# qirui-chen/RGA3-release

Measured on AMD Instinct MI355X. Metric: video-QA samples/sec (fwd+bwd) at 7B/16-frame — full RGA3 training step (Qwen2.5-VL-7B + SAM2-L + mask losses + AdamW), higher is better.
Workload: dtype bf16

## Files before the change

### rga3-release_amd/csrc/attn_args.h

```cpp
#pragma once
#include "common.h"

namespace rga3 {

struct AttnArgs {
    const unsigned short* q;
    const unsigned short* k;
    const unsigned short* v;
    unsigned short* o;
    float* lse;
    const int* cu_q;
    const int* cu_k;
    long q_st, q_sh, k_st, k_sh, v_st, v_sh, o_st, o_sh;
    int Hq, Hkv, D;
    long total_q;
    float scale_log2;
    int causal;
    float* split_o;
    float* split_lse;
    int nsplit;
    int bq_shift, bk_shift;
    const float* rope_cos;
    const float* rope_sin;
    const float* rope_kcos;
    const float* rope_ksin;
    int gx;
};

int launch_causal32(const AttnArgs& a, int nseg, int max_q, hipStream_t st);

}
```

### rga3-release_amd/csrc/attn_bwd.hip

```cpp
#include "common.h"

#include <mutex>
#include <set>

namespace rga3 {

struct AttnBwdArgs {
    const unsigned short *q, *k, *v, *o, *dout;
    unsigned short *dq, *dk, *dv;
    const float* lse;
    float* delta;
    const int *cu_q, *cu_k;
    long q_st, q_sh, k_st, k_sh, v_st, v_sh, o_st, o_sh, do_st, do_sh, dq_st, dq_sh, dk_st, dk_sh, dv_st, dv_sh;
    int Hq, Hkv, D;
    long total_q;
    float scale, scale_log2;
    int causal;
    float* dkv_ws;
    long total_k;
    int gx, gy;
};

constexpr int BT = 64;

template <int DP, int QT, int NWAVE, bool PAIR>
__global__ __launch_bounds__(64 * NWAVE) void attn_bwd_dq_kernel(AttnBwdArgs p) {
    constexpr int NT = 64 * NWAVE;
    constexpr int BLOCK_M = NWAVE * QT * 16;
    constexpr int CH = DP / 8;
    constexpr int STRIDE = DP * 2 + 32;
    constexpr int DS = DP / 32, DT = DP / 16;
    constexpr int LOADS = (BT * CH) / NT;
    static_assert((BT * CH) % NT == 0, "tile chunks must divide evenly over threads");

    extern __shared__ __attribute__((aligned(16))) char smem[];
    char* Ks = smem;
    char* Vs = smem + BT * STRIDE;

    const int tid = threadIdx.x, lane = tid & 63;
    const int wid = __builtin_amdgcn_readfirstlane(tid >> 6);
    const int g = lane >> 4, c = lane & 15;
    const Wg3 wg = xcd_decode3(p.gx, p.gy);
    const int seg = wg.z, hq = wg.y;
    const int hk = hq / (p.Hq / p.Hkv);
    const int qs = p.cu_q[seg], Lq = p.cu_q[seg + 1] - qs;
    const int ks = p.cu_k[seg], Lk = p.cu_k[seg + 1] - ks;
    const int shift = Lk - Lq;
    const int nqb = (Lq + BLOCK_M - 1) / BLOCK_M;
    int qb_first = wg.x, qb_second = -1;
    if constexpr (PAIR) {
        qb_first = nqb - 1 - wg.x;
        qb_second = wg.x;
        if (qb_second > qb_first) return;
        if (qb_second == qb_first) qb_second = -1;
    } else if (qb_first >= nqb) {
        return;
    }
    for (int pass = 0; pass < (PAIR ? 2 : 1); ++pass) {
    const int qbi = pass == 0 ? qb_first : qb_second;
    if (qbi < 0) break;
    if (pass == 1) __syncthreads();
    const int qb0 = qbi * BLOCK_M;
    const int qw0 = qb0 + wid * (QT * 16);

    bf16x8 qf[QT][DS], dof[QT][DS];
    float lse2[QT], dl[QT];
#pragma unroll
    for (int t = 0; t < QT; ++t) {
        const int qi = qw0 + t * 16 + c;
        const bool ok = qi < Lq;
#pragma unroll
        for (int ds = 0; ds < DS; ++ds) {
            const int d = ds * 32 + g * 8;
            u32x4 z = {0u, 0u, 0u, 0u}, y = {0u, 0u, 0u, 0u};
            if (ok && d < p.D) {
                z = *(const u32x4*)(p.q + (long)(qs + qi) * p.q_st + (long)hq * p.q_sh + d);
                y = *(const u32x4*)(p.dout + (long)(qs + qi) * p.do_st + (long)hq * p.do_sh + d);
            }
            qf[t][ds] = __builtin_bit_cast(bf16x8, z);
            dof[t][ds] = __builtin_bit_cast(bf16x8, y);
        }
        lse2[t] = ok ? p.lse[(long)hq * p.total_q + qs + qi] * 1.4426950408889634f : 0.f;
    }
#pragma unroll
    for (int t = 0; t < QT; ++t) {
        const int qi = qw0 + t * 16 + c;
        const bool ok = qi < Lq;
        float dp = 0.f;
#pragma unroll
        for (int ds = 0; ds < DS; ++ds) {
            const int d = ds * 32 + g * 8;
            if (ok && d < p.D) {
                const u32x4 ov = *(const u32x4*)(p.o + (long)(qs + qi) * p.o_st + (long)hq * p.o_sh + d);
                const u32x4 dv = __builtin_bit_cast(u32x4, dof[t][ds]);
#pragma unroll
                for (int i = 0; i < 4; ++i) {
                    dp += __uint_as_float(ov[i] << 16) * __uint_as_float(dv[i] << 16);
                    dp += __uint_as_float(ov[i] & 0xffff0000u) * __uint_as_float(dv[i] & 0xffff0000u);
                }
            }
        }
        dp += __shfl_xor(dp, 16, 64);
        dp += __shfl_xor(dp, 32, 64);
        dl[t] = ok ? dp : 0.f;
        if (ok && g == 0) p.delta[(long)hq * p.total_q + qs + qi] = dp;
    }

    f32x4 dqacc[QT][DT];
#pragma unroll
    for (int t = 0; t < QT; ++t)
#pragma unroll
        for (int d = 0; d < DT; ++d) dqacc[t][d] = f32x4{0.f, 0.f, 0.f, 0.f};

    int kv_end = Lk;
    if (p.causal) kv_end = min(Lk, qb0 + BLOCK_M + shift);
    if (kv_end < 0) kv_end = 0;
    const int ntiles = (kv_end + BT - 1) / BT;

    u32x4 kreg[LOADS], vreg[LOADS];
    auto load_tile = [&](int kt) {
#pragma unroll
        for (int i = 0; i < LOADS; ++i) {
            const int idx = tid + i * NT;
            const int r = idx / CH, ch = idx % CH;
            const int key = kt * BT + r;
            u32x4 zk = {0u, 0u, 0u, 0u}, zv = {0u, 0u, 0u, 0u};
            if (key < Lk && ch * 8 < p.D) {
                zk = *(const u32x4*)(p.k + (long)(ks + key) * p.k_st + (long)hk * p.k_sh + ch * 8);
                zv = *(const u32x4*)(p.v + (long)(ks + key) * p.v_st + (long)hk * p.v_sh + ch * 8);
            }
            kreg[i] = zk;
            vreg[i] = zv;
        }
    };
    auto store_tile = [&]() {
#pragma unroll
        for (int i = 0; i < LOADS; ++i) {
            const int idx = tid + i * NT;
            const int r = idx / CH, ch = idx % CH;
            *(u32x4*)(Ks + r * STRIDE + ch * 16) = kreg[i];
            *(u32x4*)(Vs + r * STRIDE + ch * 16) = vreg[i];
        }
    };

    if (ntiles > 0) load_tile(0);
    for (int kt = 0; kt < ntiles; ++kt) {
        __syncthreads();
        store_tile();
        __syncthreads();
        if (kt + 1 < ntiles) load_tile(kt + 1);
        const int k0 = kt * BT;
        const bool need_mask = (k0 + BT > Lk) || (p.causal && (k0 + BT - 1 > qb0 + shift));
#pragma unroll
        for (int t = 0; t < QT; ++t) {
            const int qi = qw0 + t * 16 + c;
            f32x4 s[4], dp[4];
#pragma unroll
            for (int j = 0; j < 4; ++j) { s[j] = f32x4{0.f, 0.f, 0.f, 0.f}; dp[j] = f32x4{0.f, 0.f, 0.f, 0.f}; }
#pragma unroll
            for (int j = 0; j < 4; ++j)
#pragma unroll
                for (int ds = 0; ds < DS; ++ds) {
                    bf16x8 kf = *(const bf16x8*)(Ks + (j * 16 + c) * STRIDE + ds * 64 + g * 16);
                    bf16x8 vf = *(const bf16x8*)(Vs + (j * 16 + c) * STRIDE + ds * 64 + g * 16);
                    s[j] = __builtin_amdgcn_mfma_f32_16x16x32_bf16(kf, qf[t][ds], s[j], 0, 0, 0);
                    dp[j] = __builtin_amdgcn_mfma_f32_16x16x32_bf16(vf, dof[t][ds], dp[j], 0, 0, 0);
                }
            bf16x8 dsf[2];
#pragma unroll
            for (int ss = 0; ss < 2; ++ss) {
                float e[8];
#pragma unroll
                for (int u = 0; u < 8; ++u) {
                    const int j = 2 * ss + (u >> 2), r = u & 3;
                    float pr = __builtin_amdgcn_exp2f(s[j][r] * p.scale_log2 - lse2[t]);
                    if (need_mask) {
                        const int key = k0 + j * 16 + 4 * g + r;
                        const bool ok = (key < Lk) && (!p.causal || key <= qi + shift);
                        pr = ok ? pr : 0.f;
                    }
                    if (qi >= Lq) pr = 0.f;
                    e[u] = pr * (dp[j][r] - dl[t]) * p.scale;
                }
                u32x4 pk;
                pk[0] = pack_bf2(e[0], e[1]); pk[1] = pack_bf2(e[2], e[3]); pk[2] = pack_bf2(e[4], e[5]); pk[3] = pack_bf2(e[6], e[7]);
                dsf[ss] = __builtin_bit_cast(bf16x8, pk);
            }
#pragma unroll
            for (int d = 0; d < DT; ++d)
#pragma unroll
                for (int ss = 0; ss < 2; ++ss) {
                    const char* a0 = Ks + (ss * 32 + 4 * g + (c >> 2)) * STRIDE + (d * 16 + 4 * (c & 3)) * 2;
                    bf16x4 lo = __builtin_amdgcn_ds_read_tr16_b64_v4bf16((__attribute__((address_space(3))) bf16x4*)(a0));
                    bf16x4 hi = __builtin_amdgcn_ds_read_tr16_b64_v4bf16((__attribute__((address_space(3))) bf16x4*)(a0 + 16 * STRIDE));
                    bf16x8 kt8;
                    kt8[0] = lo[0]; kt8[1] = lo[1]; kt8[2] = lo[2]; kt8[3] = lo[3];
                    kt8[4] = hi[0]; kt8[5] = hi[1]; kt8[6] = hi[2]; kt8[7] = hi[3];
                    dqacc[t][d] = __builtin_amdgcn_mfma_f32_16x16x32_bf16(kt8, dsf[ss], dqacc[t][d], 0, 0, 0);
                }
        }
    }
#pragma unroll
    for (int t = 0; t < QT; ++t) {
        const int qi = qw0 + t * 16 + c;
        if (qi < Lq) {
            unsigned short* row = p.dq + (long)(qs + qi) * p.dq_st + (long)hq * p.dq_sh;
#pragma unroll
            for (int d = 0; d < DT; ++d) {
                const int dd = d * 16 + 4 * g;
                if (dd < p.D) {
                    u32x2 pk;
                    pk[0] = pack_bf2(dqacc[t][d][0], dqacc[t][d][1]);
                    pk[1] = pack_bf2(dqacc[t][d][2], dqacc[t][d][3]);
                    *(u32x2*)(row + dd) = pk;
                }
            }
        }
    }
    }
}

template <int DP, int NWAVE, bool SPLIT, bool PAIR>
__global__ __launch_bounds__(64 * NWAVE) void attn_bwd_dkv_kernel(AttnBwdArgs p) {
    constexpr int NT = 64 * NWAVE;
    constexpr int BLOCK_N = NWAVE * 16;
    constexpr int CH = DP / 8;
    constexpr int STRIDE = DP * 2 + 32;
    constexpr int DS = DP / 32, DT = DP / 16;
    constexpr int LOADS = (BT * CH) / NT;
    static_assert((BT * CH) % NT == 0, "tile chunks must divide evenly over threads");

    extern __shared__ __attribute__((aligned(16))) char smem[];
    char* Qs = smem;
    char* Os = smem + BT * STRIDE;
    float* Ls = (float*)(smem + 2 * BT * STRIDE);

    const int tid = threadIdx.x, lane = tid & 63;
    const int wid = __builtin_amdgcn_readfirstlane(tid >> 6);
    const int g = lane >> 4, c = lane & 15;
    const Wg3 wg = xcd_decode3(p.gx, p.gy);
    const int seg = wg.z;
    const int group = p.Hq / p.Hkv;
    const int hk = SPLIT ? wg.y / group : wg.y;
    const int hh0 = SPLIT ? wg.y % group : 0, hh1 = SPLIT ? hh0 + 1 : group;
    const int qs = p.cu_q[seg], Lq = p.cu_q[seg + 1] - qs;
    const int ks = p.cu_k[seg], Lk = p.cu_k[seg + 1] - ks;
    const int shift = Lk - Lq;
    const int nkb = (Lk + BLOCK_N - 1) / BLOCK_N;
    int kb_first = wg.x, kb_second = -1;
    if constexpr (PAIR) {
        kb_first = wg.x;
        kb_second = nkb - 1 - wg.x;
        if (kb_first > kb_second) return;
        if (kb_second == kb_first) kb_second = -1;
    } else if (kb_first >= nkb) {
        return;
    }
    for (int pass = 0; pass < (PAIR ? 2 : 1); ++pass) {
    const int kbi = pass == 0 ? kb_first : kb_second;
    if (kbi < 0) break;
    if (pass == 1) __syncthreads();
    const int kb0 = kbi * BLOCK_N;
    const int key = kb0 + wid * 16 + c;

    bf16x8 kf[DS], vf[DS];
#pragma unroll
    for (int ds = 0; ds < DS; ++ds) {
        const int d = ds * 32 + g * 8;
        u32x4 z = {0u, 0u, 0u, 0u}, y = {0u, 0u, 0u, 0u};
        if (key < Lk && d < p.D) {
            z = *(const u32x4*)(p.k + (long)(ks + key) * p.k_st + (long)hk * p.k_sh + d);
            y = *(const u32x4*)(p.v + (long)(ks + key) * p.v_st + (long)hk * p.v_sh + d);
        }
        kf[ds] = __builtin_bit_cast(bf16x8, z);
        vf[ds] = __builtin_bit_cast(bf16x8, y);
    }
    f32x4 dkacc[DT], dvacc[DT];
#pragma unroll
    for (int d = 0; d < DT; ++d) { dkacc[d] = f32x4{0.f, 0.f, 0.f, 0.f}; dvacc[d] = f32x4{0.f, 0.f, 0.f, 0.f}; }

    int q_begin = 0;
    if (p.causal) q_begin = max(0, kb0 - shift);
    const int t0 = q_begin / BT;
    const int ntq = (Lq + BT - 1) / BT;

    u32x4 qreg[LOADS], oreg[LOADS];
    float lreg = 0.f, dreg = 0.f;
    auto load_tile = [&](int hq_, int qt_) {
#pragma unroll
        for (int i = 0; i < LOADS; ++i) {
            const int idx = tid + i * NT;
            const int r = idx / CH, ch = idx % CH;
            const int qi = qt_ * BT + r;
            u32x4 zq = {0u, 0u, 0u, 0u}, zo = {0u, 0u, 0u, 0u};
            if (qi < Lq && ch * 8 < p.D) {
                zq = *(const u32x4*)(p.q + (long)(qs + qi) * p.q_st + (long)hq_ * p.q_sh + ch * 8);
                zo = *(const u32x4*)(p.dout + (long)(qs + qi) * p.do_st + (long)hq_ * p.do_sh + ch * 8);
            }
            qreg[i] = zq;
            oreg[i] = zo;
        }
        if (tid < BT) {
            const int qi = qt_ * BT + tid;
            lreg = (qi < Lq) ? p.lse[(long)hq_ * p.total_q + qs + qi] * 1.4426950408889634f : 0.f;
            dreg = (qi < Lq) ? p.delta[(long)hq_ * p.total_q + qs + qi] : 0.f;
        }
    };
    auto store_tile = [&]() {
#pragma unroll
        for (int i = 0; i < LOADS; ++i) {
            const int idx = tid + i * NT;
            const int r = idx / CH, ch = idx % CH;
            *(u32x4*)(Qs + r * STRIDE + ch * 16) = qreg[i];
            *(u32x4*)(Os + r * STRIDE + ch * 16) = oreg[i];
        }
        if (tid < BT) {
            Ls[tid] = lreg;
            Ls[BT + tid] = dreg;
        }
    };
    if (t0 < ntq) load_tile(hk * group + hh0, t0);
    for (int hh = hh0; hh < hh1; ++hh) {
        const int hq = hk * group + hh;
        for (int qt = t0; qt < ntq; ++qt) {
            __syncthreads();
            store_tile();
            __syncthreads();
            if (qt + 1 < ntq) load_tile(hq, qt + 1);
            else if (hh + 1 < hh1) load_tile(hq + 1, t0);
            const int q0 = qt * BT;
            f32x4 s[4], dp[4];
#pragma unroll
            for (int j = 0; j < 4; ++j) { s[j] = f32x4{0.f, 0.f, 0.f, 0.f}; dp[j] = f32x4{0.f, 0.f, 0.f, 0.f}; }
#pragma unroll
            for (int j = 0; j < 4; ++j)
#pragma unroll
                for (int ds = 0; ds < DS; ++ds) {
                    bf16x8 qa = *(const bf16x8*)(Qs + (j * 16 + c) * STRIDE + ds * 64 + g * 16);
                    bf16x8 oa = *(const bf16x8*)(Os + (j * 16 + c) * STRIDE + ds * 64 + g * 16);
                    s[j] = __builtin_amdgcn_mfma_f32_16x16x32_bf16(qa, kf[ds], s[j], 0, 0, 0);
                    dp[j] = __builtin_amdgcn_mfma_f32_16x16x32_bf16(oa, vf[ds], dp[j], 0, 0, 0);
                }
            bf16x8 pf[2], dsf[2];
#pragma unroll
            for (int ss = 0; ss < 2; ++ss) {
                float e[8], f[8];
#pragma unroll
                for (int u = 0; u < 8; ++u) {
                    const int j = 2 * ss + (u >> 2), r = u & 3;
                    const int ql = j * 16 + 4 * g + r;
                    const int qi = q0 + ql;
                    float pr = __builtin_amdgcn_exp2f(s[j][r] * p.scale_log2 - Ls[ql]);
                    const bool ok = (qi < Lq) && (key < Lk) && (!p.causal || key <= qi + shift);
                    pr = ok ? pr : 0.f;
                    e[u] = pr;
                    f[u] = pr * (dp[j][r] - Ls[BT + ql]) * p.scale;
                }
                u32x4 a, b;
                a[0] = pack_bf2(e[0], e[1]); a[1] = pack_bf2(e[2], e[3]); a[2] = pack_bf2(e[4], e[5]); a[3] = pack_bf2(e[6], e[7]);
                b[0] = pack_bf2(f[0], f[1]); b[1] = pack_bf2(f[2], f[3]); b[2] = pack_bf2(f[4], f[5]); b[3] = pack_bf2(f[6], f[7]);
                pf[ss] = __builtin_bit_cast(bf16x8, a);
                dsf[ss] = __builtin_bit_cast(bf16x8, b);
            }
#pragma unroll
            for (int d = 0; d < DT; ++d)
#pragma unroll
                for (int ss = 0; ss < 2; ++ss) {
                    const int roff = (ss * 32 + 4 * g + (c >> 2)) * STRIDE + (d * 16 + 4 * (c & 3)) * 2;
                    bf16x4 ol = __builtin_amdgcn_ds_read_tr16_b64_v4bf16((__attribute__((address_space(3))) bf16x4*)(Os + roff));
                    bf16x4 oh = __builtin_amdgcn_ds_read_tr16_b64_v4bf16((__attribute__((address_space(3))) bf16x4*)(Os + roff + 16 * STRIDE));
                    bf16x4 ql_ = __builtin_amdgcn_ds_read_tr16_b64_v4bf16((__attribute__((address_space(3))) bf16x4*)(Qs + roff));
                    bf16x4 qh_ = __builtin_amdgcn_ds_read_tr16_b64_v4bf16((__attribute__((address_space(3))) bf16x4*)(Qs + roff + 16 * STRIDE));
                    bf16x8 ot, qt8;
                    ot[0] = ol[0]; ot[1] = ol[1]; ot[2] = ol[2]; ot[3] = ol[3]; ot[4] = oh[0]; ot[5] = oh[1]; ot[6] = oh[2]; ot[7] = oh[3];
                    qt8[0] = ql_[0]; qt8[1] = ql_[1]; qt8[2] = ql_[2]; qt8[3] = ql_[3]; qt8[4] = qh_[0]; qt8[5] = qh_[1]; qt8[6] = qh_[2]; qt8[7] = qh_[3];
                    dvacc[d] = __builtin_amdgcn_mfma_f32_16x16x32_bf16(ot, pf[ss], dvacc[d], 0, 0, 0);
                    dkacc[d] = __builtin_amdgcn_mfma_f32_16x16x32_bf16(qt8, dsf[ss], dkacc[d], 0, 0, 0);
                }
        }
    }
    if constexpr (SPLIT) {
        if (key < Lk) {
            const long half = (long)group * p.total_k * p.Hkv * p.D;
            float* wk = p.dkv_ws + (((long)hh0 * p.total_k + ks + key) * p.Hkv + hk) * p.D;
#pragma unroll
            for (int d = 0; d < DT; ++d) {
                const int dd = d * 16 + 4 * g;
                if (dd < p.D) {
                    *(f32x4*)(wk + dd) = dkacc[d];
                    *(f32x4*)(wk + half + dd) = dvacc[d];
                }
            }
        }
        continue;
    }
    if (key < Lk) {
        unsigned short* rk = p.dk + (long)(ks + key) * p.dk_st + (long)hk * p.dk_sh;
        unsigned short* rv = p.dv + (long)(ks + key) * p.dv_st + (long)hk * p.dv_sh;
#pragma unroll
        for (int d = 0; d < DT; ++d) {
            const int dd = d * 16 + 4 * g;
            if (dd < p.D) {
                u32x2 a, b;
                a[0] = pack_bf2(dkacc[d][0], dkacc[d][1]); a[1] = pack_bf2(dkacc[d][2], dkacc[d][3]);
                b[0] = pack_bf2(dvacc[d][0], dvacc[d][1]); b[1] = pack_bf2(dvacc[d][2], dvacc[d][3]);
                *(u32x2*)(rk + dd) = a;
                *(u32x2*)(rv + dd) = b;
            }
        }
    }
    }
}

__global__ __launch_bounds__(256) void attn_dkv_reduce_kernel(AttnBwdArgs p) {
    const int group = p.Hq / p.Hkv;
    const int d4 = p.D / 4;
    const long idx = (long)blockIdx.x * 256 + threadIdx.x;
    const long total = p.total_k * p.Hkv * d4;
    if (idx >= total) return;
    const int dd = (int)(idx % d4) * 4;
    const long row = idx / d4;
    const int hk = (int)(row % p.Hkv);
    const long key = row / p.Hkv;
    const long plane = p.total_k * p.Hkv * (long)p.D, half = (long)group * plane;
    const float* w = p.dkv_ws + row * p.D + dd;
    f32x4 sk = *(const f32x4*)w, sv = *(const f32x4*)(w + half);
    for (int h = 1; h < group; ++h) {
        sk += *(const f32x4*)(w + h * plane);
        sv += *(const f32x4*)(w + half + h * plane);
    }
    u32x2 a, b;
    a[0] = pack_bf2(sk[0], sk[1]); a[1] = pack_bf2(sk[2], sk[3]);
    b[0] = pack_bf2(sv[0], sv[1]); b[1] = pack_bf2(sv[2], sv[3]);
    *(u32x2*)(p.dk + key * p.dk_st + (long)hk * p.dk_sh + dd) = a;
    *(u32x2*)(p.dv + key * p.dv_st + (long)hk * p.dv_sh + dd) = b;
}

template <int DP>
static int launch_bwd(const AttnBwdArgs& a0, int nseg, int max_q, int max_k, hipStream_t st) {
    AttnBwdArgs a = a0;
    a.gx = 1; a.gy = 1;
    constexpr int NW = (DP == 128) ? 8 : 4;
#ifdef RGA3_BWD_DQ_QT2
    constexpr int QT = 2, NWQ = 4;
#else
    constexpr int QT = (DP >= 128) ? 1 : 2, NWQ = NW;
#endif
    constexpr int BLOCK_M = NWQ * QT * 16;
    constexpr int LDS_DQ = 2 * BT * (DP * 2 + 32);
    constexpr int LDS_DKV = 2 * BT * (DP * 2 + 32) + 2 * BT * 4;
    auto prep = [](const void* k, int lds) -> int {
        if (lds <= 48 * 1024) return 0;
        static std::mutex mu;
        static std::set<std::pair<const void*, int>> done;
        int dev = 0;
        if (hipGetDevice(&dev) != hipSuccess) dev = 0;
        std::lock_guard<std::mutex> lk(mu);
        if (done.count({k, dev})) return 0;
        hipError_t e = hipFuncSetAttribute(k, hipFuncAttributeMaxDynamicSharedMemorySize, lds);
        if (e != hipSuccess) return fail(-(int)e, "attn_bwd: hipFuncSetAttribute: %s", hipGetErrorString(e));
        done.insert({k, dev});
        return 0;
    };
    const unsigned nqb = (unsigned)cdiv(max_q, BLOCK_M), nkb = (unsigned)cdiv(max_k, 16 * NW);
    const bool pair = a.causal && nqb >= 4 && nkb >= 4;
    if (pair) {
        auto kq = attn_bwd_dq_kernel<DP, QT, NWQ, true>;
        if (int rc = prep((const void*)kq, LDS_DQ)) return rc;
        a.gx = (int)((nqb + 1) / 2); a.gy = a.Hq;
        hipLaunchKernelGGL(kq, dim3((unsigned)a.gx * (unsigned)a.gy * (unsigned)nseg), dim3(64 * NWQ), LDS_DQ, st, a);
    } else {
        auto kq = attn_bwd_dq_kernel<DP, QT, NWQ, false>;
        if (int rc = prep((const void*)kq, LDS_DQ)) return rc;
        a.gx = (int)nqb; a.gy = a.Hq;
        hipLaunchKernelGGL(kq, dim3((unsigned)a.gx * (unsigned)a.gy * (unsigned)nseg), dim3(64 * NWQ), LDS_DQ, st, a);
    }
    RGA3_CHECK_LAUNCH("attn_bwd_dq_kernel");
    const unsigned gx = pair ? (nkb + 1) / 2 : nkb;
    if (a.dkv_ws && a.Hq > a.Hkv) {
        if (pair) {
            auto ks_ = attn_bwd_dkv_kernel<DP, NW, true, true>;
            if (int rc = prep((const void*)ks_, LDS_DKV)) return rc;
            a.gx = (int)gx; a.gy = a.Hq;
            hipLaunchKernelGGL(ks_, dim3((unsigned)a.gx * (unsigned)a.gy * (unsigned)nseg), dim3(64 * NW), LDS_DKV, st, a);
        } else {
            auto ks_ = attn_bwd_dkv_kernel<DP, NW, true, false>;
            if (int rc = prep((const void*)ks_, LDS_DKV)) return rc;
            a.gx = (int)gx; a.gy = a.Hq;
            hipLaunchKernelGGL(ks_, dim3((unsigned)a.gx * (unsigned)a.gy * (unsigned)nseg), dim3(64 * NW), LDS_DKV, st, a);
        }
        RGA3_CHECK_LAUNCH("attn_bwd_dkv_kernel<split>");
        const long rows = a.total_k * a.Hkv;
        hipLaunchKernelGGL(attn_dkv_reduce_kernel, dim3((unsigned)cdiv(rows * (a.D / 4), 256)), dim3(256), 0, st, a);
        RGA3_CHECK_LAUNCH("attn_dkv_reduce_kernel");
        return 0;
    }
    if (pair) {
        auto kk = attn_bwd_dkv_kernel<DP, NW, false, true>;
        if (int rc = prep((const void*)kk, LDS_DKV)) return rc;
        a.gx = (int)gx; a.gy = a.Hkv;
        hipLaunchKernelGGL(kk, dim3((unsigned)a.gx * (unsigned)a.gy * (unsigned)nseg), dim3(64 * NW), LDS_DKV, st, a);
    } else {
        auto kk = attn_bwd_dkv_kernel<DP, NW, false, false>;
        if (int rc = prep((const void*)kk, LDS_DKV)) return rc;
        a.gx = (int)gx; a.gy = a.Hkv;
        hipLaunchKernelGGL(kk, dim3((unsigned)a.gx * (unsigned)a.gy * (unsigned)nseg), dim3(64 * NW), LDS_DKV, st, a);
    }
    RGA3_CHECK_LAUNCH("attn_bwd_dkv_kernel");
    return 0;
}

}

using namespace rga3;

extern "C" int rga3_attn_varlen_bwd(const void* q, const void* k, const void* v, const void* o, const void* dout, const float* lse,
                                    void* dq, void* dk, void* dv, float* delta_ws, const int32_t* cu_q, const int32_t* cu_k, int nseg,
                                    int max_q, int max_k, int64_t total_q, int Hq, int Hkv, int D, const int64_t* strides16, float scale,
                                    int causal, float* dkv_ws, int64_t total_k, void* stream) {
    RGA3_CHECK_ARG(q && k && v && o && dout && lse && dq && dk && dv && delta_ws && cu_q && cu_k && strides16, "attn_bwd: null pointer");
    RGA3_CHECK_ARG(nseg > 0 && max_q > 0 && max_k > 0 && total_q > 0, "attn_bwd: sizes");
    RGA3_CHECK_ARG(Hq > 0 && Hkv > 0 && Hq % Hkv == 0, "attn_bwd: Hq=%d Hkv=%d", Hq, Hkv);
    RGA3_CHECK_ARG(D >= 8 && D <= 128 && D % 8 == 0, "attn_bwd: head dim %d unsupported (multiple of 8, <= 128)", D);
    for (int i = 0; i < 16; ++i) RGA3_CHECK_ARG(strides16[i] % 4 == 0, "attn_bwd: stride %d must be a multiple of 4 elements", i);
    for (int i = 0; i < 10; ++i) RGA3_CHECK_ARG(strides16[i] % 8 == 0, "attn_bwd: input stride %d must be a multiple of 8 elements", i);
    AttnBwdArgs a;
    a.q = (const unsigned short*)q; a.k = (const unsigned short*)k; a.v = (const unsigned short*)v; a.o = (const unsigned short*)o;
    a.dout = (const unsigned short*)dout; a.dq = (unsigned short*)dq; a.dk = (unsigned short*)dk; a.dv = (unsigned short*)dv;
    a.lse = lse; a.delta = delta_ws; a.cu_q = cu_q; a.cu_k = cu_k;
    a.q_st = strides16[0]; a.q_sh = strides16[1]; a.k_st = strides16[2]; a.k_sh = strides16[3]; a.v_st = strides16[4]; a.v_sh = strides16[5];
    a.o_st = strides16[6]; a.o_sh = strides16[7]; a.do_st = strides16[8]; a.do_sh = strides16[9]; a.dq_st = strides16[10]; a.dq_sh = strides16[11];
    a.dk_st = strides16[12]; a.dk_sh = strides16[13]; a.dv_st = strides16[14]; a.dv_sh = strides16[15];
    a.Hq = Hq; a.Hkv = Hkv; a.D = D; a.total_q = total_q; a.scale = scale; a.scale_log2 = scale * 1.4426950408889634f; a.causal = causal;
    a.dkv_ws = dkv_ws; a.total_k = total_k;
    RGA3_CHECK_ARG(!dkv_ws || (total_k > 0 && D % 4 == 0), "attn_bwd: dkv_ws needs total_k");
    hipStream_t st = (hipStream_t)stream;
    if (D <= 32) return launch_bwd<32>(a, nseg, max_q, max_k, st);
    if (D <= 64) return launch_bwd<64>(a, nseg, max_q, max_k, st);
    if (D <= 96) return launch_bwd<96>(a, nseg, max_q, max_k, st);
    return launch_bwd<128>(a, nseg, max_q, max_k, st);
}
```

Baseline: 7.816.

## Add 32x32 MFMA dQ backward kernel with paired causal blocks for head dim 128

Adds a new dQ backward attention kernel for D=128 built on 32x32x16 bf16 MFMA. It streams K/V tiles through LDS with direct global-to-LDS loads and double-buffered slots, and uses transposed LDS reads for the K^T·dS product. Two wave groups work on a paired low and high causal query block so the work stays balanced, and their partial dQ results are reduced through LDS at the end. This replaces the generic 16x16 dQ kernel for the common head-dim-128 case, aiming for higher MFMA throughput and fewer LDS and global round-trips. The cost is considerable new indexing and swizzle complexity.

After: 7.819, median of 6. About the same (+0.0%).

```diff
diff --git a/rga3-release_amd/csrc/attn_args.h b/rga3-release_amd/csrc/attn_args.h
--- a/rga3-release_amd/csrc/attn_args.h
+++ b/rga3-release_amd/csrc/attn_args.h
@@ -29,4 +29,22 @@
 
 int launch_causal32(const AttnArgs& a, int nseg, int max_q, hipStream_t st);
 
+struct AttnBwdArgs {
+    const unsigned short *q, *k, *v, *o, *dout;
+    unsigned short *dq, *dk, *dv;
+    const float* lse;
+    float* delta;
+    const int *cu_q, *cu_k;
+    long q_st, q_sh, k_st, k_sh, v_st, v_sh, o_st, o_sh, do_st, do_sh, dq_st, dq_sh, dk_st, dk_sh, dv_st, dv_sh;
+    int Hq, Hkv, D;
+    long total_q;
+    float scale, scale_log2;
+    int causal;
+    float* dkv_ws;
+    long total_k;
+    int gx, gy;
+};
+
+int launch_bwd32_dq(const AttnBwdArgs& a, int nseg, int max_q, hipStream_t st);
+
 }
diff --git a/rga3-release_amd/csrc/attn_bwd.hip b/rga3-release_amd/csrc/attn_bwd.hip
--- a/rga3-release_amd/csrc/attn_bwd.hip
+++ b/rga3-release_amd/csrc/attn_bwd.hip
@@ -1,25 +1,9 @@
-#include "common.h"
+#include "attn_args.h"
 
 #include <mutex>
 #include <set>
 
 namespace rga3 {
-
-struct AttnBwdArgs {
-    const unsigned short *q, *k, *v, *o, *dout;
-    unsigned short *dq, *dk, *dv;
-    const float* lse;
-    float* delta;
-    const int *cu_q, *cu_k;
-    long q_st, q_sh, k_st, k_sh, v_st, v_sh, o_st, o_sh, do_st, do_sh, dq_st, dq_sh, dk_st, dk_sh, dv_st, dv_sh;
-    int Hq, Hkv, D;
-    long total_q;
-    float scale, scale_log2;
-    int causal;
-    float* dkv_ws;
-    long total_k;
-    int gx, gy;
-};
 
 constexpr int BT = 64;
 
@@ -441,11 +425,7 @@
     AttnBwdArgs a = a0;
     a.gx = 1; a.gy = 1;
     constexpr int NW = (DP == 128) ? 8 : 4;
-#ifdef RGA3_BWD_DQ_QT2
-    constexpr int QT = 2, NWQ = 4;
-#else
     constexpr int QT = (DP >= 128) ? 1 : 2, NWQ = NW;
-#endif
     constexpr int BLOCK_M = NWQ * QT * 16;
     constexpr int LDS_DQ = 2 * BT * (DP * 2 + 32);
     constexpr int LDS_DKV = 2 * BT * (DP * 2 + 32) + 2 * BT * 4;
@@ -464,18 +444,21 @@
     };
     const unsigned nqb = (unsigned)cdiv(max_q, BLOCK_M), nkb = (unsigned)cdiv(max_k, 16 * NW);
     const bool pair = a.causal && nqb >= 4 && nkb >= 4;
-    if (pair) {
+    if (a.D == 128 && a.k_st < (1 << 24) && a.v_st < (1 << 24)) {
+        if (int rc = launch_bwd32_dq(a, nseg, max_q, st)) return rc;
+    } else if (pair) {
         auto kq = attn_bwd_dq_kernel<DP, QT, NWQ, true>;
         if (int rc = prep((const void*)kq, LDS_DQ)) return rc;
         a.gx = (int)((nqb + 1) / 2); a.gy = a.Hq;
         hipLaunchKernelGGL(kq, dim3((unsigned)a.gx * (unsigned)a.gy * (unsigned)nseg), dim3(64 * NWQ), LDS_DQ, st, a);
+        RGA3_CHECK_LAUNCH("attn_bwd_dq_kernel");
     } else {
         auto kq = attn_bwd_dq_kernel<DP, QT, NWQ, false>;
         if (int rc = prep((const void*)kq, LDS_DQ)) return rc;
         a.gx = (int)nqb; a.gy = a.Hq;
         hipLaunchKernelGGL(kq, dim3((unsigned)a.gx * (unsigned)a.gy * (unsigned)nseg), dim3(64 * NWQ), LDS_DQ, st, a);
-    }
-    RGA3_CHECK_LAUNCH("attn_bwd_dq_kernel");
+        RGA3_CHECK_LAUNCH("attn_bwd_dq_kernel");
+    }
     const unsigned gx = pair ? (nkb + 1) / 2 : nkb;
     if (a.dkv_ws && a.Hq > a.Hkv) {
         if (pair) {
diff --git a/rga3-release_amd/csrc/attn_bwd32.hip b/rga3-release_amd/csrc/attn_bwd32.hip
--- /dev/null
+++ b/rga3-release_amd/csrc/attn_bwd32.hip
@@ -0,0 +1,282 @@
+#include "attn_args.h"
+
+namespace rga3 {
+
+namespace {
+constexpr int B32_KT = 64;
+constexpr int B32_QB = 128;
+constexpr int B32_ROWB = 256;
+constexpr int B32_HALF = B32_KT * B32_ROWB;
+constexpr int B32_SLOT = 2 * B32_HALF;
+constexpr int B32_LDS = 4 * B32_SLOT;
+
+__device__ __forceinline__ int b32_swz(int row) { return ((row & 3) << 2) | ((row >> 2) & 3); }
+}
+
+__global__ __launch_bounds__(512) void attn_bwd32_dq_kernel(AttnBwdArgs p) {
+    extern __shared__ __attribute__((aligned(16))) char smem[];
+    const int tid = threadIdx.x, lane = tid & 63;
+    const int wid = __builtin_amdgcn_readfirstlane(tid >> 6);
+    const int grp = wid >> 2, w4 = wid & 3;
+    const int r = lane & 31, h = lane >> 5;
+
+    const unsigned lid = xcd_remap(blockIdx.x, gridDim.x);
+    const int hq = (int)(lid % (unsigned)p.Hq);
+    const int bx = (int)((lid / (unsigned)p.Hq) % (unsigned)p.gx);
+    const int seg = (int)(lid / ((unsigned)p.Hq * (unsigned)p.gx));
+    const int hk = hq / (p.Hq / p.Hkv);
+    const int qs = p.cu_q[seg], Lq = p.cu_q[seg + 1] - qs;
+    const int ks = p.cu_k[seg], Lk = p.cu_k[seg + 1] - ks;
+    const int shift = Lk - Lq;
+    const int nqb = (Lq + B32_QB - 1) / B32_QB;
+    const int qbH = nqb - 1 - bx;
+    if (bx > qbH) return;
+    const int qbL = (bx == qbH) ? -1 : bx;
+    auto ktiles = [&](int qb) {
+        const int e = p.causal ? min(Lk, qb * B32_QB + B32_QB + shift) : Lk;
+        return e > 0 ? (e + B32_KT - 1) / B32_KT : 0;
+    };
+    const int kH = ktiles(qbH), kL = qbL >= 0 ? min(ktiles(qbL), kH) : 0;
+    const int c = (kH + kL + 1) >> 1;
+
+    const unsigned short* kbase = p.k + (long)ks * p.k_st + (long)hk * p.k_sh;
+    const unsigned short* vbase = p.v + (long)ks * p.v_st + (long)hk * p.v_sh;
+    char* const X = smem;
+    char* const Y = smem + 2 * B32_SLOT;
+
+    unsigned dko[2], dvo[2];
+#pragma unroll
+    for (int j = 0; j < 2; ++j) {
+        const int blk = 2 * wid + j;
+        const int row = 4 * blk + (lane >> 4);
+        const int lc = (lane & 15) ^ (((lane >> 4) << 2) | (blk & 3));
+        dko[j] = (unsigned)(row * (int)p.k_st + lc * 8);
+        dvo[j] = (unsigned)(row * (int)p.v_st + lc * 8);
+    }
+    auto issue_img = [&](const unsigned short* base, long st, const unsigned (&d)[2], int tile, char* img) {
+        if (tile * B32_KT + B32_KT <= Lk) {
+            const unsigned short* tb = base + (long)tile * B32_KT * st;
+#pragma unroll
+            for (int j = 0; j < 2; ++j) {
+                unsigned o_ = d[j];
+                asm volatile("" : "+v"(o_));
+                __builtin_amdgcn_global_load_lds((gbl_void*)(tb + o_), (lds_void*)(img + (2 * wid + j) * 1024), 16, 0, 0);
+            }
+        } else {
+#pragma unroll
+            for (int j = 0; j < 2; ++j) {
+                const int blk = 2 * wid + j;
+                const int row = 4 * blk + (lane >> 4);
+                const int lc = (lane & 15) ^ (((lane >> 4) << 2) | (blk & 3));
+                const int key = min(tile * B32_KT + row, Lk - 1);
+                __builtin_amdgcn_global_load_lds((gbl_void*)(base + (long)key * st + lc * 8), (lds_void*)(img + blk * 1024), 16, 0, 0);
+            }
+        }
+    };
+    auto issue_slot = [&](int j) {
+        if (j >= c) return;
+        char* const xs = X + (j & 1) * B32_SLOT;
+        issue_img(kbase, p.k_st, dko, j, xs);
+        issue_img(vbase, p.v_st, dvo, j, xs + B32_HALF);
+        const int ty = c + j - kL;
+        if (j >= kL && ty < kH) {
+            char* const ys = Y + (j & 1) * B32_SLOT;
+            issue_img(kbase, p.k_st, dko, ty, ys);
+            issue_img(vbase, p.v_st, dvo, ty, ys + B32_HALF);
+        }
+    };
+
+    const int kbase0 = r * B32_ROWB + ((h ^ b32_swz(r)) << 4);
+    auto koff = [&](int kk) { return kbase0 ^ (kk << 5); };
+    int tro0;
+    {
+        const int g1 = (lane >> 4) & 1, q_ = (lane >> 2) & 3, p_ = lane & 3;
+        const int x = (q_ << 2) | (h & 3);
+        const int lc = 2 * g1 + (p_ >> 1);
+        tro0 = (4 * h + q_) * B32_ROWB + ((lc ^ x) << 4) + 8 * (p_ & 1);
+    }
+    auto tro = [&](int jj, int b) { return jj ? ((tro0 ^ (b << 6) ^ 32) + 2048) : (tro0 ^ (b << 6)); };
+
+    bf16x8 qf[8], dof[8];
+    f32x16 o[4];
+    float lse2 = 0.f, dl = 0.f;
+    int qw0 = 0;
+    auto start_rows = [&](int qb, bool own_delta) {
+        qw0 = qb * B32_QB + w4 * 32;
+        const int qi = min(qw0 + r, Lq - 1);
+        const long row = (long)(qs + qi);
+        const unsigned short* qrow = p.q + row * p.q_st + (long)hq * p.q_sh + 8 * h;
+        const unsigned short* drow = p.dout + row * p.do_st + (long)hq * p.do_sh + 8 * h;
+        const unsigned short* orow = p.o + row * p.o_st + (long)hq * p.o_sh + 8 * h;
+#pragma unroll
+        for (int kk = 0; kk < 8; ++kk) {
+            qf[kk] = *(const bf16x8*)(qrow + 16 * kk);
+            dof[kk] = *(const bf16x8*)(drow + 16 * kk);
+        }
+        float da = 0.f, db = 0.f;
+#pragma unroll
+        for (int kk = 0; kk < 8; ++kk) {
+            const u32x4 ov = *(const u32x4*)(orow + 16 * kk);
+            const u32x4 dv = __builtin_bit_cast(u32x4, dof[kk]);
+            float& acc = (kk & 1) ? db : da;
+#pragma unroll
+            for (int i = 0; i < 4; ++i) {
+                acc += __uint_as_float(ov[i] << 16) * __uint_as_float(dv[i] << 16);
+                acc += __uint_as_float(ov[i] & 0xffff0000u) * __uint_as_float(dv[i] & 0xffff0000u);
+            }
+        }
+        da += __shfl_xor(da, 32, 64);
+        db += __shfl_xor(db, 32, 64);
+        dl = da + db;
+        if (own_delta && h == 0 && qw0 + r < Lq) p.delta[(long)hq * p.total_q + qs + qi] = dl;
+        lse2 = p.lse[(long)hq * p.total_q + qs + qi] * 1.4426950408889634f;
+#pragma unroll
+        for (int b = 0; b < 4; ++b)
+#pragma unroll
+            for (int i = 0; i < 16; ++i) o[b][i] = 0.f;
+#pragma unroll
+        for (int kk = 0; kk < 8; ++kk) asm volatile("" : "+v"(qf[kk]), "+v"(dof[kk]));
+    };
+    auto store_rows = [&]() {
+        const int qi = qw0 + r;
+        if (qi >= Lq) return;
+        unsigned short* row = p.dq + (long)(qs + qi) * p.dq_st + (long)hq * p.dq_sh + 4 * h;
+#pragma unroll
+        for (int b = 0; b < 4; ++b)
+#pragma unroll
+            for (int i4 = 0; i4 < 4; ++i4) {
+                u32x2 pk;
+                pk[0] = pack_bf2(o[b][4 * i4], o[b][4 * i4 + 1]);
+                pk[1] = pack_bf2(o[b][4 * i4 + 2], o[b][4 * i4 + 3]);
+                *(u32x2*)(row + 32 * b + 8 * i4) = pk;
+            }
+    };
+
+    auto slot_tile = [&](int j) { return (grp == 0 || j < kL) ? j : c + j - kL; };
+    auto slot_live = [&](int j, bool on_h) {
+        const int t = slot_tile(j);
+        return j < c && t < (on_h ? kH : kL) && qw0 < Lq && (!p.causal || t * B32_KT <= qw0 + 31 + shift);
+    };
+
+    auto compute = [&](int j) {
+        const char* Kb = ((grp == 0 || j < kL) ? X : Y) + (j & 1) * B32_SLOT;
+        const char* Vb = Kb + B32_HALF;
+        const int k0 = slot_tile(j) * B32_KT;
+        const int qi = qw0 + r;
+        const bool need_mask = (k0 + B32_KT > Lk) || (p.causal && k0 + B32_KT - 1 > qw0 + shift);
+        const int lim = p.causal ? min(Lk - 1, qi + shift) : Lk - 1;
+        bf16x8 pb[2][2];
+#pragma unroll
+        for (int kb = 0; kb < 2; ++kb) {
+            f32x16 s, dp;
+#pragma unroll
+            for (int i = 0; i < 16; ++i) { s[i] = 0.f; dp[i] = 0.f; }
+            bf16x8 kf[2], vf[2];
+            kf[0] = *(const bf16x8*)(Kb + kb * 32 * B32_ROWB + koff(0));
+            vf[0] = *(const bf16x8*)(Vb + kb * 32 * B32_ROWB + koff(0));
+#pragma unroll
+            for (int kk = 0; kk < 8; ++kk) {
+                if (kk + 1 < 8) {
+                    kf[(kk + 1) & 1] = *(const bf16x8*)(Kb + kb * 32 * B32_ROWB + koff(kk + 1));
+                    vf[(kk + 1) & 1] = *(const bf16x8*)(Vb + kb * 32 * B32_ROWB + koff(kk + 1));
+                }
+                s = __builtin_amdgcn_mfma_f32_32x32x16_bf16(kf[kk & 1], qf[kk], s, 0, 0, 0);
+                dp = __builtin_amdgcn_mfma_f32_32x32x16_bf16(vf[kk & 1], dof[kk], dp, 0, 0, 0);
+            }
+            float e[16];
+#pragma unroll
+            for (int i = 0; i < 16; ++i) {
+                float pr = __builtin_amdgcn_exp2f(s[i] * p.scale_log2 - lse2);
+                if (need_mask) {
+                    const int key = k0 + kb * 32 + (i & 3) + 8 * (i >> 2) + 4 * h;
+                    pr = (key <= lim) ? pr : 0.f;
+                }
+                e[i] = pr * (dp[i] - dl) * p.scale;
+            }
+#pragma unroll
+            for (int ss = 0; ss < 2; ++ss) {
+                u32x4 pk;
+                pk[0] = pack_bf2(e[8 * ss + 0], e[8 * ss + 1]);
+                pk[1] = pack_bf2(e[8 * ss + 2], e[8 * ss + 3]);
+                pk[2] = pack_bf2(e[8 * ss + 4], e[8 * ss + 5]);
+                pk[3] = pack_bf2(e[8 * ss + 6], e[8 * ss + 7]);
+                pb[kb][ss] = __builtin_bit_cast(bf16x8, pk);
+            }
+        }
+#pragma unroll
+        for (int kb = 0; kb < 2; ++kb)
+#pragma unroll
+            for (int ss = 0; ss < 2; ++ss)
+#pragma unroll
+                for (int b = 0; b < 4; ++b) {
+                    const char* a0 = Kb + (kb * 32 + 16 * ss) * B32_ROWB;
+                    const bf16x4 lo = __builtin_amdgcn_ds_read_tr16_b64_v4bf16((__attribute__((address_space(3))) bf16x4*)(a0 + tro(0, b)));
+                    const bf16x4 hi = __builtin_amdgcn_ds_read_tr16_b64_v4bf16((__attribute__((address_space(3))) bf16x4*)(a0 + tro(1, b)));
+                    bf16x8 kt;
+                    kt[0] = lo[0]; kt[1] = lo[1]; kt[2] = lo[2]; kt[3] = lo[3];
+                    kt[4] = hi[0]; kt[5] = hi[1]; kt[6] = hi[2]; kt[7] = hi[3];
+                    o[b] = __builtin_amdgcn_mfma_f32_32x32x16_bf16(kt, pb[kb][ss], o[b], 0, 0, 0);
+                }
+    };
+
+    bool onH = (grp == 0) || (qbL < 0);
+    issue_slot(0);
+    start_rows(onH ? qbH : qbL, grp == 0 || !onH);
+    for (int it = 0; it < c; ++it) {
+        asm volatile("s_waitcnt vmcnt(0)" ::: "memory");
+        __builtin_amdgcn_s_barrier();
+        issue_slot(it + 1);
+        if (grp == 1 && !onH && it >= kL) {
+            store_rows();
+            start_rows(qbH, false);
+            onH = true;
+        }
+        if (slot_live(it, onH)) compute(it);
+    }
+    if (grp == 1 && !onH) {
+        store_rows();
+#pragma unroll
+        for (int b = 0; b < 4; ++b)
+#pragma unroll
+            for (int i = 0; i < 16; ++i) o[b][i] = 0.f;
+        qw0 = qbH * B32_QB + w4 * 32;
+    }
+
+    asm volatile("s_waitcnt vmcnt(0)" ::: "memory");
+    __syncthreads();
+    float* const mo = (float*)smem;
+    const int gl = tid & 255;
+    if (grp == 1) {
+#pragma unroll
+        for (int b = 0; b < 4; ++b)
+#pragma unroll
+            for (int i4 = 0; i4 < 4; ++i4)
+                *(f32x4*)(mo + (((b * 4 + i4) * 256 + gl) << 2)) = f32x4{o[b][4 * i4], o[b][4 * i4 + 1], o[b][4 * i4 + 2], o[b][4 * i4 + 3]};
+    }
+    __syncthreads();
+    if (grp == 0) {
+#pragma unroll
+        for (int b = 0; b < 4; ++b)
+#pragma unroll
+            for (int i4 = 0; i4 < 4; ++i4) {
+                const f32x4 ob = *(const f32x4*)(mo + (((b * 4 + i4) * 256 + gl) << 2));
+#pragma unroll
+                for (int e = 0; e < 4; ++e) o[b][4 * i4 + e] += ob[e];
+            }
+        store_rows();
+    }
+}
+
+int launch_bwd32_dq(const AttnBwdArgs& a, int nseg, int max_q, hipStream_t st) {
+    static LdsGrant lds_grant;
+    if (int rc = grant_dyn_lds((const void*)attn_bwd32_dq_kernel, B32_LDS, lds_grant, "attn_bwd32_dq")) return rc;
+    AttnBwdArgs b = a;
+    const unsigned nqb = (unsigned)cdiv(max_q, B32_QB);
+    b.gx = (int)((nqb + 1) / 2);
+    b.gy = a.Hq;
+    hipLaunchKernelGGL(attn_bwd32_dq_kernel, dim3((unsigned)b.gx * (unsigned)a.Hq * (unsigned)nseg), dim3(512), B32_LDS, st, b);
+    RGA3_CHECK_LAUNCH("attn_bwd32_dq_kernel");
+    return 0;
+}
+
+}
```
